# kije/HSLU_I.BA_RAYTRACING.F2501_raytracer

Hardware: AMD Instinct MI355X
Metric: Mray/s (primary+secondary, rays counted as the reference casts them), semesterbild@high_resolution (higher is better)
Workload: dtype f32; 1 GPU; semesterbild@high_resolution+anti_aliasing+soft_shadows (text.obj); width=1620, height=1350, rays_per_frame=34992000, rays_traced_per_frame=19683000, pixels_written=1768966, objects=14578, lights=50, parallelism=tiles48x48/1gpu, frames_in_flight=2, build_id=6bfb61b4c07ed2fe-p0s0w0o6, queue_bytes=0, scene_budget_bytes=2147483648, phases=0

## Files before the change

### hslu_i/ba_raytracing/f2501_raytracer_amd/csrc/rt_api.cpp

```cpp
#include <hip/hip_runtime.h>

#include <algorithm>
#include <chrono>
#include <cmath>
#include <cstdio>
#include <cstdlib>
#include <cstring>
#include <string>
#include <vector>

#include "rt_cell_prune.h"
#include "rt_host.h"

static void trace_point(hipStream_t stream, const char* what, uint32_t a = 0, uint32_t b = 0, uint32_t c = 0);
#define RC_TRY(expr) do { const int rc_ = (expr); if (rc_ != RT_OK) return rc_; } while (0)

extern "C" {

#ifndef RT_BUILD_ID
#define RT_BUILD_ID "unknown"
#endif
const char* rt_build_id(void) { return RT_BUILD_ID; }

int rt_selftest_exact_math(int device, const float* in, float* out_sqrt, float* out_rcp, uint32_t n) {
// ... 26 lines not shown
void rt_scene_destroy(rt_scene* s) {
  if (!s) return;
  (void)hipSetDevice(s->device);
  if (s->tables_ev) (void)hipEventDestroy(s->tables_ev);
  for (hipEvent_t e : s->frame_ev)
    if (e) (void)hipEventDestroy(e);
  for (auto& w : s->ws) {
    if (w.cnt_ev) (void)hipEventDestroy(w.cnt_ev);
    if (w.cnt_host) (void)hipHostFree(w.cnt_host);
    if (w.fork_ev) (void)hipEventDestroy(w.fork_ev);
    w.acc.release();
    for (auto& l : w.lane) {
      if (l.stream) (void)hipStreamSynchronize(l.stream), (void)hipStreamDestroy(l.stream);
      if (l.done_ev) (void)hipEventDestroy(l.done_ev);
      for (int k = 0; k < 2; k++) {
        if (l.shade_stream[k]) (void)hipStreamSynchronize(l.shade_stream[k]), (void)hipStreamDestroy(l.shade_stream[k]);
        if (l.shade_done[k]) (void)hipEventDestroy(l.shade_done[k]);
      }
      for (hipEvent_t e : l.level_ev) (void)hipEventDestroy(e);
      if (l.hit_ev) (void)hipEventDestroy(l.hit_ev);
      for (DevBuf* b : {&l.queues, &l.qcount, &l.trace_ws, &l.hard, &l.hitrec, &l.sets}) b->release();
    }
  }
  for (DevBuf* b : {&s->blob, &s->aa, &s->cloud, &s->counters, &s->suplist, &s->fb, &s->aux_rgb, &s->costmap, &s->aux_id, &s->aux_t, &s->flag_geo, &s->flags, &s->cell_lists, &s->progress_fb, &s->rays_argb})
    b->release();
  rt_scene_release_update(s);
  delete s;
}

static int upload(DevBuf& b, const void* src, size_t bytes) {
  int rc = b.ensure(bytes);
  if (rc != RT_OK) return rc;
  if (bytes) {
    hipError_t e = hipMemcpy(b.p, src, bytes, hipMemcpyHostToDevice);
    if (e != hipSuccess) return fail(RT_ERR_HIP, "hipMemcpy H2D failed: %s", hipGetErrorString(e));
  }
  return RT_OK;
}

int rt_scene_create(const rt_scene_desc* d, int device, rt_scene** out) {
  if (!d || !out) return fail(RT_ERR_INVALID_ARG, "null argument");
  *out = nullptr;
  int rc = rt_check_scene_desc(d);
  if (rc != RT_OK) return rc;
  if ((rc = rt_open_device(device)) != RT_OK) return rc;

  rt_scene* s = new rt_scene();
  s->device = device;
// ... 23 lines not shown
  s->n_tri_cells = pk.n_tri_cells;
  s->bytes_bvh = pk.bytes_bvh;
  s->max_leaf = pk.max_leaf;
  memcpy(s->aabb_lo, pk.aabb_lo, sizeof(s->aabb_lo));
  memcpy(s->aabb_hi, pk.aabb_hi, sizeof(s->aabb_hi));
  *out = s;
  return RT_OK;
}

int rt_scene_bvh_info(const rt_scene* s, rt_bvh_info* out) {
  if (!s || !out) return fail(RT_ERR_INVALID_ARG, "null argument");
  *out = s->info;
  return RT_OK;
}

int rt_scene_memory_info(const rt_scene* s, rt_scene_info* out) {
  if (!s || !out) return fail(RT_ERR_INVALID_ARG, "null argument");
  memset(out, 0, sizeof(*out));
  out->bytes_bvh = s->bytes_bvh;
  out->bytes_geometry = s->blob.cap > s->bytes_bvh ? s->blob.cap - s->bytes_bvh : 0;
  out->bytes_flags = s->flags.cap + s->flag_geo.cap;
  out->bytes_cell_lists = s->cell_lists.cap;
  out->bytes_tables = s->aa.cap + s->cloud.cap + s->counters.cap + s->suplist.cap + s->costmap.cap;
  for (const auto& w : s->ws) {
    out->bytes_workspace += w.bytes();
    for (const auto& l : w.lane) out->bytes_workspace += l.qcount.cap;
  }
  out->bytes_frames = s->fb.cap + s->aux_rgb.cap + s->aux_id.cap + s->aux_t.cap + s->progress_fb.cap + s->rays_argb.cap;
  out->bytes_total = out->bytes_geometry + out->bytes_bvh + out->bytes_flags + out->bytes_cell_lists + out->bytes_tables + out->bytes_workspace +
                     out->bytes_frames;
  out->budget_bytes = s->budget;
  out->n_receiver_cells = s->n_cells;
  out->cell_lists_built = s->cell_lists_built ? 1u : 0u;
  return RT_OK;
}

}

int rt_validate_params(const rt_params* p) {
  if (!p) return fail(RT_ERR_INVALID_ARG, "null params");
  if (p->abi_version != RT_ABI_VERSION)
    return fail(RT_ERR_INVALID_ARG, "rt_params.abi_version %u != %u", p->abi_version, RT_ABI_VERSION);
  if (p->width == 0 || p->height == 0) return fail(RT_ERR_INVALID_ARG, "empty frame");
  if ((uint64_t)p->width * p->height > 0x7FFFFFFFull) return fail(RT_ERR_INVALID_ARG, "frame too large");
  if (p->win_w && (p->win_x0 + (uint64_t)p->win_w > p->width || p->win_y0 + (uint64_t)p->win_h > p->height || !p->win_h))
    return fail(RT_ERR_INVALID_ARG, "window outside the frame");
// ... 90 lines not shown
  const size_t n = (size_t)p->n_cloud_sets * P->light_mult * 3;
  const bool new_table = s->cloud_host.size() != n || memcmp(s->cloud_host.data(), p->cloud_sets, n * 4) != 0;
  const bool new_scale = s->cloud_ball_f[0] != p->fw || s->cloud_ball_f[1] != p->fh || s->cloud_ball_f[2] != p->fd;
  if (new_table || new_scale) {
    RC_TRY(up.begin());
    RC_TRY(s->cloud.ensure(n / 3 * 16));
    if (new_table) s->cloud_host.assign(p->cloud_sets, p->cloud_sets + n);
    s->cloud_ball_f[0] = p->fw, s->cloud_ball_f[1] = p->fh, s->cloud_ball_f[2] = p->fd;
    rt_scale_cloud(s->cloud_host.data(), n, s->cloud_ball_f, &s->cloud_scaled, s->cloud_ball);
    HIP_TRY(hipMemcpyAsync(s->cloud.p, s->cloud_scaled.data(), n / 3 * 16, hipMemcpyHostToDevice, up.stream));
  }
  P->cloud_sets = (const float4*)s->cloud.p;
  memcpy(P->cloud_centre, s->cloud_ball, 12);
  P->cloud_delta = s->cloud_ball[3];
  rt_beam_constants(p->eps_distance, P);
  const uint32_t cap = p->tuning.shadow_candidate_cap;
  P->cand_cap = cap == RT_CAND_CAP_NONE ? 0u : (cap ? cap : 64u);
  return RT_OK;
}

static int prepare_receiver_flags(rt_scene* s, const rt_params* p, TableUpload& up, RtDevParams* P) {
  hipStream_t stream = up.stream;
  P->recv_flags = nullptr;
  if (p->tuning.no_receiver_flags || P->cand_cap == 0u) s->notes |= RT_NOTE_RECV_FLAGS_OFF_TUNING;
  if (!s->n_cells || !(P->cloud_delta > 0.0f)) s->notes |= RT_NOTE_RECV_FLAGS_OFF_SCENE;
  if (s->dev.n_lights > 8u) s->notes |= RT_NOTE_RECV_FLAGS_OFF_LIGHTS;
  if (p->traversal != RT_TRAVERSAL_BVH) s->notes |= RT_NOTE_RECV_FLAGS_OFF_TRAVERSAL;
  if (p->flags & RT_FLAG_BACKFACE_CULLING) s->notes |= RT_NOTE_RECV_FLAGS_OFF_CULLING;
  if (!p->tuning.no_receiver_flags && P->cand_cap != 0u && s->n_cells && s->dev.n_lights <= 8u && p->traversal == RT_TRAVERSAL_BVH &&
      !(p->flags & RT_FLAG_BACKFACE_CULLING) && P->cloud_delta > 0.0f) {
    const float key[8] = {P->beam_delta, p->eps_distance, P->cloud_centre[0], P->cloud_centre[1], P->cloud_centre[2], 1.f, 0.f, 0.f};
    if (memcmp(key, s->flags_key, sizeof(key)) != 0) {
      RC_TRY(up.begin());
      RtDevParams B = *P;
      B.flag_out = (uint16_t*)s->flags.p;
      B.flag_geo = (const float4*)s->flag_geo.p;
      B.n_cells = s->n_cells;
      B.n_tri_cells = s->n_tri_cells;
      s->cell_lists_built = false;
      B.cell_list_out = nullptr;
      const size_t list_bytes = (size_t)s->n_cells * s->dev.n_lights * 16u;
      size_t free_b = 0, total_b = 0;
      const size_t flag_bytes = s->flags.cap + s->flag_geo.cap;
      if (s->dev.n_slots <= 65533u && flag_bytes + list_bytes <= s->budget && hipMemGetInfo(&free_b, &total_b) == hipSuccess &&
          list_bytes <= (free_b + s->cell_lists.cap) / 4 && s->cell_lists.ensure(list_bytes + 64) == RT_OK) {
        HIP_TRY(hipMemsetAsync(s->cell_lists.p, 0xFF, list_bytes, stream));
        B.cell_list_out = (uint16_t*)s->cell_lists.p;
        s->cell_lists_built = true;
      }
      if (!s->cell_lists_built) s->cell_lists.release();
      hipError_t e = (hipError_t)rt_launch_flags(s->dev, B, stream);
      if (e != hipSuccess) return fail(RT_ERR_HIP, "rt_flags_kernel launch failed: %s", hipGetErrorString(e));
      trace_point(stream, "rt_flags_kernel: cells, lights, lists", s->n_cells, s->dev.n_lights, s->cell_lists_built ? 1u : 0u);
      static const char* const prune_env = getenv("RT_CELL_PRUNE");
      static const bool prune_off = prune_env && *prune_env == '0';
      if (s->cell_lists_built && !prune_off) {
        RtCellPruneArgs a{};
        a.flag_geo = (const float*)s->flag_geo.p;
        a.lists = (uint16_t*)s->cell_lists.p;
        a.flags = (uint16_t*)s->flags.p;
        a.n_cells = s->n_cells, a.n_tri_cells = s->n_tri_cells;
        memcpy(a.cloud_centre, P->cloud_centre, 12);
        a.beam_delta = P->beam_delta, a.beam_eps_o = P->beam_eps_o;
        a.mode = RT_PRUNE_FULL;
        e = (hipError_t)rt_launch_cell_prune(s->dev, a, stream);
        if (e != hipSuccess) return fail(RT_ERR_HIP, "rt_cell_prune_kernel launch failed: %s", hipGetErrorString(e));
        trace_point(stream, "rt_cell_prune_kernel: cells, lights", s->n_cells, s->dev.n_lights, 0u);
      }
      memcpy(s->flags_key, key, sizeof(key));
    }
    P->recv_flags = (const uint16_t*)s->flags.p;
    if (s->cell_lists_built && !p->tuning.no_cell_lists) P->cell_lists = (const uint4*)s->cell_lists.p;
  }
  if (!P->cell_lists) s->notes |= RT_NOTE_CELL_LISTS_OFF;
  return RT_OK;
}

static void copy_frame_shape(rt_scene* s, const rt_params* p, uint32_t* argb_dev, const rt_aux* aux_dev, RtDevParams* P) {
  P->max_depth_reflection = p->max_depth_reflection;
  P->max_depth_refraction = p->max_depth_refraction;
  s->sort_bits_wanted = p->tuning.sort_bits;
  s->lanes_wanted = p->tuning.sub_frames;
  s->phases_wanted = p->tuning.phases;
  s->levels_wanted = p->tuning.levels;
  if (p->win_w) {
    P->win_x0 = p->win_x0, P->win_y0 = p->win_y0, P->win_w = p->win_w, P->win_h = p->win_h;
  } else {
    P->win_x0 = P->win_y0 = 0;
    P->win_w = p->width;
    P->win_h = p->height;
// ... 782 lines not shown
```

### hslu_i/ba_raytracing/f2501_raytracer_amd/csrc/rt_cell_prune.h

```cpp
#pragma once

#include "rt_refit.h"

#define RT_PRUNE_LIST_SLOTS 8u
#define RT_PRUNE_LIST_END 0xFFFFu
#define RT_PRUNE_LIST_OVERFLOW 0xFFFEu
#define RT_PRUNE_G 8e-6f

#define RT_PRUNE_FAR 1u
#define RT_PRUNE_EUCLID 2u
#define RT_PRUNE_NO_RHO_WC 4u
#define RT_PRUNE_NO_RHO_FAR 8u
#define RT_PRUNE_FULL (RT_PRUNE_FAR | RT_PRUNE_EUCLID)

struct RtCellPruneArgs {
  const float* flag_geo;
  uint16_t* lists;
  uint16_t* flags;
  uint32_t n_cells, n_tri_cells;
  float cloud_centre[3];
  float beam_delta, beam_eps_o;
  uint32_t mode;
};

struct RtPruneBeam {
  float p[3], c[3], dseg[3];
  float rho, delta, lenp;
};

RT_HD static inline float rt_prune_dot(const float a[3], const float b[3]) {
  return rt_fadd(rt_fadd(rt_fmul(a[0], b[0]), rt_fmul(a[1], b[1])), rt_fmul(a[2], b[2]));
}
RT_HD static inline void rt_prune_cross(const float a[3], const float b[3], float out[3]) {
  out[0] = rt_fadd(rt_fmul(a[1], b[2]), -rt_fmul(a[2], b[1]));
  out[1] = rt_fadd(rt_fmul(a[2], b[0]), -rt_fmul(a[0], b[2]));
  out[2] = rt_fadd(rt_fmul(a[0], b[1]), -rt_fmul(a[1], b[0]));
}
RT_HD static inline void rt_prune_sub(const float a[3], const float b[3], float out[3]) {
  out[0] = rt_fadd(a[0], -b[0]), out[1] = rt_fadd(a[1], -b[1]), out[2] = rt_fadd(a[2], -b[2]);
}
RT_HD static inline float rt_prune_norm1(const float a[3]) { return rt_fadd(rt_fadd(fabsf(a[0]), fabsf(a[1])), fabsf(a[2])); }
RT_HD static inline float rt_prune_norm(const float a[3]) {
  const float q = rt_prune_dot(a, a);
  return q > 1e-30f ? rt_fmul(rt_fsqrt(q), 1.00001f) : rt_prune_norm1(a);
}
// ... 118 lines not shown
}

RT_HD static inline void rt_cell_prune_cell(const RtDevScene& sc, const char* base, const RtCellPruneArgs& a, uint32_t c, uint16_t* list, uint16_t* flag) {
  float pm[3], pt[8][3], extra;
  if (!rt_prune_cell_hull(sc, base, a, c, pm, pt, &extra)) return;
  float r = 0.0f, scale = rt_fadd(rt_prune_norm1(pm), extra);
  for (int k = 0; k < 8; k++) {
    float dk[3];
    rt_prune_sub(pt[k], pm, dk);
    r = fmaxf(r, rt_prune_norm(dk));
    scale = fmaxf(scale, rt_fadd(rt_prune_norm1(pt[k]), extra));
  }
  RtPruneBeam B;
  B.p[0] = pm[0], B.p[1] = pm[1], B.p[2] = pm[2];
  B.rho = rt_fadd(rt_fadd(rt_fmul(r, 1.0001f), rt_fmul(2e-6f, scale)), a.beam_eps_o);
  const float* lights = (const float*)(base + sc.off_lights);
  const float* isect = (const float*)(base + sc.off_tri_isect);
  uint32_t fl = *flag;
  bool fl_changed = false;
  for (uint32_t l = 0; l < sc.n_lights && l < 8u; l++) {
    uint16_t* w = list + (size_t)l * RT_PRUNE_LIST_SLOTS;
    uint16_t in[RT_PRUNE_LIST_SLOTS];
    memcpy(in, __builtin_assume_aligned(w, 16), 16);
    if (in[0] >= RT_PRUNE_LIST_OVERFLOW) continue;
    for (int x = 0; x < 3; x++) B.c[x] = rt_fadd(lights[8u * l + x], a.cloud_centre[x]);
    rt_prune_sub(B.c, B.p, B.dseg);
    B.delta = rt_fadd(a.beam_delta, rt_fmul(2e-6f, rt_fadd(scale, rt_prune_norm1(B.c))));
    B.lenp = rt_fadd(rt_fadd(rt_prune_norm(B.dseg), B.delta), B.rho);
    uint32_t n = 0, n_in = 0;
    uint16_t out[RT_PRUNE_LIST_SLOTS];
    for (uint32_t k = 0; k < RT_PRUNE_LIST_SLOTS; k++) {
      const uint32_t slot = in[k];
      if (slot >= RT_PRUNE_LIST_OVERFLOW) break;
      n_in++;
      if (slot < sc.n_slots && rt_prune_rule(B, isect + 12u * (size_t)slot, a.mode)) continue;
      out[n++] = (uint16_t)slot;
    }
    if (n == n_in) continue;
    for (uint32_t k = n; k < RT_PRUNE_LIST_SLOTS; k++) out[k] = (uint16_t)RT_PRUNE_LIST_END;
    memcpy(__builtin_assume_aligned(w, 16), out, 16);
    if (n == 0u) fl |= 1u << l, fl_changed = true;
  }
  if (fl_changed) *flag = (uint16_t)fl;
}

struct RtPackedScene;
void rt_cell_prune_packed(const RtPackedScene& pk, RtCellPruneArgs a);
int rt_launch_cell_prune(const RtDevScene& sc, const RtCellPruneArgs& a, void* stream);
```

### hslu_i/ba_raytracing/f2501_raytracer_amd/csrc/rt_host.h

```cpp
#pragma once

#include <hip/hip_runtime.h>

#include <string>
#include <vector>

#include "rt_ray_key.h"
#include "rt_scene_pack.h"

#define fail rt_fail

#define HIP_TRY(expr)                                                                          \
  do {                                                                                         \
    hipError_t e_ = (expr);                                                                    \
    if (e_ != hipSuccess)                                                                      \
      return fail(e_ == hipErrorOutOfMemory ? RT_ERR_OOM : RT_ERR_HIP, "%s failed: %s", #expr, \
                  hipGetErrorString(e_));                                                      \
  } while (0)

#define RT_SLOTS 4
#define RT_LANES 2
#define RT_MAX_DEPTH 64u

#define RT_CNT_OVERFLOW 0u
// ... 227 lines not shown
  uint32_t key_gen = 0;
  uint32_t sticky_notes = 0;
  bool stream_verified = false;
  uint32_t est[RT_LANES][RT_CNT_STRIDE] = {{0}};
  bool est_valid = false;
  uint32_t sort_bits_wanted = 0;
  uint32_t lanes_wanted = 0;
  uint32_t phases_wanted = 0;
  uint32_t levels_wanted = 0;
  uint32_t calm_frames = 1u << 30;
  uint32_t tables_version = 0;
  float aabb_lo[3] = {0.f, 0.f, 0.f}, aabb_hi[3] = {1.f, 1.f, 1.f};
  std::vector<float> aa_host, cloud_host, cloud_scaled;
  std::vector<uint32_t> aa_table;
  uint32_t aa_unique = 0;
  bool aa_dedup = true;
  hipEvent_t tables_ev = nullptr;
  hipStream_t tables_stream = nullptr, last_stream = nullptr;
  bool tables_pending = false, rendered = false;
  float cloud_ball[4] = {0.f, 0.f, 0.f, -1.f};
  DevBuf flag_geo, flags;
  DevBuf cell_lists;
  bool cell_lists_built = false;
  uint32_t n_cells = 0, n_tri_cells = 0;
  float flags_key[8] = {-1.f, 0.f, 0.f, 0.f, 0.f, 0.f, 0.f, 0.f};
  float cloud_ball_f[3] = {0.f, 0.f, 0.f};
  hipEvent_t frame_ev[RT_SLOTS] = {};
  bool frame_pending[RT_SLOTS] = {};
  uint32_t frame_seq[RT_SLOTS] = {};
  hipStream_t frame_stream[RT_SLOTS] = {};
  uint32_t frame_no = 0;
  int cur_block = 0, last_block = 0;
  int cur_ws = 0;
  int ws_last_block[RT_SLOTS] = {0, 1, 2, 3};
  uint32_t notes = 0;
  size_t queue_bytes = 0;
  RtRefitPlan plan;
  DevBuf plan_dev, upd_dev;
  size_t plan_off[5] = {0, 0, 0, 0, 0};
  void* upd_stage = nullptr;
  size_t upd_stage_cap = 0;
  float* upd_back = nullptr;
  uint64_t sah_created[2] = {0, 0};
  float sah_tri_cost = 2.0f;
  DevBuf sah_dev;
  uint32_t max_leaf = 4;
// ... 39 lines not shown
```

### hslu_i/ba_raytracing/f2501_raytracer_amd/csrc/rt_internal.h

```cpp
#pragma once

#include <stdint.h>

#include <vector>

#include "../../../../include/rt_hip.h"


struct RtNode {
  float lo0[3];
  uint32_t c0;
  float hi0[3];
  uint32_t n0;
  float lo1[3];
  uint32_t c1;
  float hi1[3];
  uint32_t n1;
};
static_assert(sizeof(RtNode) == 64, "node must be 64 bytes");

struct RtThrNode {
  float lo[3];
  uint32_t skip;
  float hi[3];
// ... 190 lines not shown
    case 10u: return lists ? RT_PRIMARY_SOFT10 : RT_PRIMARY_SOFT10_FLAGS;
    case 19u: return lists ? RT_PRIMARY_SOFT19 : RT_PRIMARY_SOFT19_FLAGS;
    case 28u: return lists ? RT_PRIMARY_SOFT28 : RT_PRIMARY_SOFT28_FLAGS;
    default: return RT_PRIMARY_GENERIC;
  }
}
static inline const char* rt_primary_variant_name(int v) {
  static const char* const names[RT_PRIMARY_VARIANTS] = {"rt_primary_kernel", "rt_primary_soft10_kernel", "rt_primary_soft19_kernel",
                                                         "rt_primary_soft28_kernel", "rt_primary_soft10_flags_kernel",
                                                         "rt_primary_soft19_flags_kernel", "rt_primary_soft28_flags_kernel"};
  return v >= 0 && v < RT_PRIMARY_VARIANTS ? names[v] : "";
}

uint32_t rt_primary_pixels_per_wg(const RtDevParams& p);
uint32_t rt_primary_total_wgs(const RtDevParams& p);
int rt_launch_primary(const RtDevScene& sc, const RtDevParams& p, uint32_t n_wgs, void* stream);
int rt_primary_variant_used(const RtDevScene& sc, const RtDevParams& p);
int rt_launch_trace(const RtDevScene& sc, const RtDevParams& p, uint32_t n_wgs, void* stream);
int rt_launch_sort(const RtDevParams& p, uint32_t n_wgs_place, void* stream);
int rt_launch_shade(const RtDevScene& sc, const RtDevParams& p, uint32_t n_wgs, void* stream);
int rt_launch_hard(const RtDevScene& sc, const RtDevParams& p, uint32_t n_wgs, void* stream);
int rt_launch_resolve(const RtDevParams& p, void* stream);
int rt_launch_flags(const RtDevScene& sc, const RtDevParams& p, void* stream);
int rt_launch_hit(const RtDevScene& sc, const RtDevParams& p, uint32_t n_wgs, void* stream);
int rt_launch_classify(const RtDevScene& sc, const RtDevParams& p, bool level0, uint32_t n_wgs, void* stream);
int rt_launch_compact(const RtDevParams& p, uint32_t n_wgs, void* stream);
int rt_launch_sets(const RtDevScene& sc, const RtDevParams& p, bool level0, int cls, uint32_t n_wgs, void* stream);
bool rt_has_cost_kernel();
bool rt_phases_arrive_inline();
int rt_launch_selftest_math(const float* in, float* out_sqrt, float* out_rcp, uint32_t n, void* stream);
int rt_launch_scatter(uint32_t* argb, const uint32_t* recv, const uint32_t* rank_off, const uint32_t* tile_slot, uint32_t width,
                      uint32_t height, uint32_t tile_size, uint32_t tiles_x, uint32_t n_ranks, void* stream);
```

### hslu_i/ba_raytracing/f2501_raytracer_amd/csrc/rt_kernels.hip

```cpp
#include <hip/hip_runtime.h>

#include <stdlib.h>

#include <type_traits>

#include "rt_internal.h"

#define RT_EPS 1.1920929e-7f

#define RT_OPAQUE(v) asm volatile("" : "+v"(v))
#define RT_OPAQUE_S(v) asm volatile("" : "+s"(v))
typedef const __attribute__((address_space(4))) char* rt_kernarg_ptr;
__device__ __forceinline__ rt_kernarg_ptr kernarg_fresh() {
  rt_kernarg_ptr p = (rt_kernarg_ptr)__builtin_amdgcn_kernarg_segment_ptr();
  asm volatile("" : "+s"(p));
  return p;
}
#define RT_KERNARG_OFF_P ((sizeof(RtDevScene) + alignof(RtDevParams) - 1) / alignof(RtDevParams) * alignof(RtDevParams))
static_assert(RT_KERNARG_OFF_P == 88, "RtDevParams follows RtDevScene at kernarg offset 88");
__device__ __forceinline__ const RtDevScene& kernarg_scene() { return *(const RtDevScene*)(const char*)kernarg_fresh(); }
__device__ __forceinline__ const RtDevParams& kernarg_params() {
  return *(const RtDevParams*)((const char*)kernarg_fresh() + RT_KERNARG_OFF_P);
}
#define wave_ballot(pred) __builtin_amdgcn_ballot_w64((bool)(pred))
// ... 668 lines not shown
    walk(std::true_type{});
  else
    walk(std::false_type{});
  return best;
}

#define RT_MAX_CANDIDATES 64u
#define RT_CAND_OVERFLOW 0xFFFFFFFFu

struct CandList {
  uint32_t reg;
  uint32_t count;
  uint32_t spheres;
  unsigned long long umbra;
#if RT_PROFILE == 5
  uint32_t own;
#endif
};

struct FatBeam {
  float r;
  V3 pt[8];
  uint16_t* list;
};
#define RT_CELL_LIST_SLOTS 8u
#define RT_CELL_LIST_END 0xFFFFu
#define RT_CELL_LIST_OVERFLOW 0xFFFEu
enum { COLLECT_OWN = 0, COLLECT_FLAGS = 1 };

template <bool CULL, int MODE = COLLECT_OWN, class C = CfgGeneric>
__device__ __forceinline__ CandList collect_light_candidates(const RtDevScene& sc, WaveCtx& W, bool alive, V3 p, V3 c,
                                                              const RtDevParams& P, V3 p_first, float p_spread, uint32_t cand_cap,
                                                              const FatBeam* fb = nullptr, bool walk_tris = true,
                                                              bool have_pre = false, uint32_t pre_reg = 0, uint32_t pre_count = 0) {
  RT_OPAQUE_S(cand_cap);
  const float delta = MODE == COLLECT_FLAGS ? P.beam_delta + fb->r : P.beam_delta;
  const float delta_e5 = MODE == COLLECT_FLAGS ? P.beam_delta_e5 + fb->r : P.beam_delta_e5;
  CandList L;
  L.reg = 0;
  L.count = 0;
  L.spheres = 0xFFFFFFFFu;
  L.umbra = 0ull;
#if RT_PROFILE == 5
  L.own = 0;
#endif
  const uint32_t lane_id = threadIdx.x & 63u;
  V3 dseg = c - p;
  float len = fmaxf(mag(dseg), 1e-20f);
  V3 inv = mk(clampf(__builtin_amdgcn_rcpf(dseg.x), -1e30f, 1e30f), clampf(__builtin_amdgcn_rcpf(dseg.y), -1e30f, 1e30f),
              clampf(__builtin_amdgcn_rcpf(dseg.z), -1e30f, 1e30f));
  V3 noi = mk(-(p.x * inv.x), -(p.y * inv.y), -(p.z * inv.z));
  V3 dl = mk(delta * fabsf(inv.x), delta * fabsf(inv.y), delta * fabsf(inv.z));
  float send = 1.0f + delta_e5 * __builtin_amdgcn_rcpf(len) + 1e-5f;
  float sbeg = -(delta_e5 * __builtin_amdgcn_rcpf(len) + 1e-5f);
  const V3 cn = noi - dl, cf = noi + dl;
  auto box = [&](const float* lo, const float* hi, float& smin) {
// ... 46 lines not shown
        rej &= wave_ballot(__builtin_fmaf(4e-6f, sk, __builtin_fmaf(X1, p_ulp, xk)) < rhs);
      }
    } else {
      rej = wave_ballot(__builtin_fmaf(4e-6f, st0, __builtin_fmaf(X1, p_ulp, xbs)) < t_push * (ad - dslack));
    }
    if (!(lanes & (open | ~rej))) return true;
    V3 y = mk((c2.y * dseg.z) + (-c2.z * dseg.y), (c2.z * dseg.x) + (-c2.x * dseg.z), (c2.x * dseg.y) + (-c2.y * dseg.x));
    float E2 = fabsf(c2.x) + fabsf(c2.y) + fabsf(c2.z);
    float ybs = __uint_as_float(__float_as_uint(dot(y, b)) ^ sgn);
    float su = E2 * geo;
    rej |= wave_ballot(ybs + su < 0.0f);
    if (!(lanes & (open | ~rej))) return true;
    V3 z = mk((dseg.y * c1.z) + (-dseg.z * c1.y), (dseg.z * c1.x) + (-dseg.x * c1.z), (dseg.x * c1.y) + (-dseg.y * c1.x));
    float E1 = fabsf(c1.x) + fabsf(c1.y) + fabsf(c1.z);
    float zbs = __uint_as_float(__float_as_uint(dot(z, b)) ^ sgn);
    float sv = E1 * geo;
    rej |= wave_ballot(zbs + sv < 0.0f) | wave_ballot((ybs + zbs) - ad - (su + sv) - dslack - 2e-6f * ad > 0.0f);
    if (!(lanes & (open | ~rej))) return true;
    if (MODE == COLLECT_FLAGS) {
      const lanemask surv = lanes & (open | ~rej);
      L.umbra |= surv;
      if (fb->list && lane_of(surv)) {
        if (L.reg < RT_CELL_LIST_SLOTS) fb->list[L.reg] = (uint16_t)slot;
        L.reg++;
      }
      return true;
    }
    if (!CULL && !(sload<uint32_t>(sc, sc.off_tri_id + slot * 4u) & RT_TRI_TRANSMISSIVE)) {
      const float dlo = ad - dslack;
      const float r_hi = lenp * __builtin_amdgcn_rcpf(dlo) * 1.00001f;
      const float r_lo = (len - delta) * __builtin_amdgcn_rcpf(ad + dslack) * 0.99999f;
      const float ex = __builtin_fmaf(4e-6f, st0, X1 * p_ulp);
      const float g_t = 2e-6f * (st0 + X1 * eps_o) * r_hi;
      const float t_lo = (xbs - ex) * r_lo - 1.001f * eps_o - g_t;
      const float t_hi = (xbs + ex) * r_hi + g_t;
      const lanemask inside = wave_ballot(ybs - su > 0.0f) & wave_ballot(zbs - sv > 0.0f) &
                              wave_ballot((ybs + zbs) + (su + sv) < dlo * 0.99999f) & wave_ballot(xbs > ex) & wave_ballot(t_lo > 2e-7f) &
                              wave_ballot(t_hi < (len - delta) - 1.01f * eps_o - 3e-7f * lenp) &
                              wave_ballot(dlo * rcp_lenp > __builtin_fmaf(2e-6f, X1, 2e-7f));
      L.umbra |= lanes & ~open & inside;
    }
#if RT_PROFILE == 5
    if (lane_of(lanes & (open | ~rej))) L.own++;
#endif
    return false;
  };
// ... 1283 lines not shown
    }
    if (any) {
      wrote = true;
      P1.argb[out_index(P1, pm2.gx, pm2.gy, pix)] = pack_argb(color);
      if (P1.aux_rgb) {
        P1.aux_rgb[3 * (size_t)pix + 0] = color.x;
        P1.aux_rgb[3 * (size_t)pix + 1] = color.y;
        P1.aux_rgb[3 * (size_t)pix + 2] = color.z;
      }
    }
  }
  if (COST && P1.cost_map && (threadIdx.x & 63u) == 0) {
    const unsigned long long dt = __builtin_readcyclecounter() - lds_cnt[16 + (threadIdx.x >> 6)];
    const uint32_t ppw = wave_local ? 4u * ppwave : 256u / n_thr;
    const uint32_t g = rt_batch_wg(P1, blockIdx.x) * ppw + (wave_local ? (threadIdx.x >> 6) * ppwave : threadIdx.x / n_thr), sup_slot = g >> 8;
    if (sup_slot < P1.n_sup) atomicAdd(&P1.cost_map[P1.sup_list ? P1.sup_list[sup_slot] : sup_slot], (uint32_t)(dt >> 6));
  }
  wave_flush(wv, P1, (uint32_t)__popcll(wave_ballot(wrote)), lds_cnt);
}

#ifndef RT_MIN_WAVES
#define RT_MIN_WAVES 6
#endif
__global__ __launch_bounds__(256, RT_MIN_WAVES) void rt_primary_kernel(RtDevScene sc, RtDevParams P) {
  __shared__ float4 lds_rgbh[256];
  __shared__ __attribute__((aligned(16))) float lds_stash[RT_STASH_FIX * 256];
  __shared__ unsigned long long lds_cnt[20];
  if (P.flags & RT_FLAG_BACKFACE_CULLING)
    primary_body<true, false>(sc, P, lds_rgbh, lds_stash, lds_cnt);
  else
    primary_body<false, false>(sc, P, lds_rgbh, lds_stash, lds_cnt);
}

#define RT_PRIMARY_SOFT_KERNEL(name, n, tables)                                                              \
  __global__ __launch_bounds__(256, RT_MIN_WAVES) void name(RtDevScene sc, RtDevParams P) {                  \
    __shared__ float4 lds_rgbh[256];                                                                         \
    __shared__ __attribute__((aligned(16))) float lds_stash[RT_STASH_FIX * 256];                             \
    __shared__ unsigned long long lds_cnt[20];                                                               \
    primary_body<false, false, false, false, CfgSoft<n, tables>>(sc, P, lds_rgbh, lds_stash, lds_cnt);       \
  }
RT_PRIMARY_SOFT_KERNEL(rt_primary_soft10_kernel, 10u, CFG_TABLES_LISTS)
RT_PRIMARY_SOFT_KERNEL(rt_primary_soft19_kernel, 19u, CFG_TABLES_LISTS)
RT_PRIMARY_SOFT_KERNEL(rt_primary_soft28_kernel, 28u, CFG_TABLES_LISTS)
RT_PRIMARY_SOFT_KERNEL(rt_primary_soft10_flags_kernel, 10u, CFG_TABLES_FLAGS)
RT_PRIMARY_SOFT_KERNEL(rt_primary_soft19_flags_kernel, 19u, CFG_TABLES_FLAGS)
RT_PRIMARY_SOFT_KERNEL(rt_primary_soft28_flags_kernel, 28u, CFG_TABLES_FLAGS)
// ... 407 lines not shown
  if (i >= P.win_w * P.win_h) return;
  const uint32_t gx = P.win_x0 + i % P.win_w, gy = P.win_y0 + i / P.win_w;
  const uint32_t pix = gy * P.width + gx;
  long long* a = P.acc + 4 * (size_t)pix;
  long long r = a[0], g = a[1], b = a[2], f = a[3];
  unsigned long long wrote = 0;
  if (f) {
    V3 c = mk((float)r * RT_ACC_INV_SCALE, (float)g * RT_ACC_INV_SCALE, (float)b * RT_ACC_INV_SCALE);
    P.argb[out_index(P, gx, gy, pix)] = pack_argb(c);
    if (P.aux_rgb) {
      P.aux_rgb[3 * (size_t)pix + 0] = c.x;
      P.aux_rgb[3 * (size_t)pix + 1] = c.y;
      P.aux_rgb[3 * (size_t)pix + 2] = c.z;
    }
    a[0] = a[1] = a[2] = a[3] = 0;
    wrote = 1;
  }
  if (P.resolve_counts_written && P.counters) {
    const uint32_t nw = (uint32_t)__popcll(wave_ballot(wrote != 0ull));
    if (nw && (threadIdx.x & 63u) == 0) atomicAdd(&P.counters[(size_t)(blockIdx.x % RT_COUNTER_REPLICAS) * 16u + 4u], (unsigned long long)nw);
  }
}

__global__ __launch_bounds__(256) void rt_flags_kernel(RtDevScene sc, RtDevParams P) {
  const uint32_t c = blockIdx.x * 256u + threadIdx.x;
  const bool have = c < P.n_cells;
  FatBeam fb;
  V3 pm = mk(0.0f, 0.0f, 0.0f);
  bool active = false;
  if (have && c < P.n_tri_cells) {
    uint32_t lo = 0u, hi = sc.n_triangles;
    while (hi - lo > 1u) {
      const uint32_t mid = (lo + hi) >> 1;
      if (__float_as_uint(P.flag_geo[3u * mid + 1u].w) <= c) lo = mid; else hi = mid;
    }
    const uint32_t t = lo;
    const float4 g0 = P.flag_geo[3u * t], g1 = P.flag_geo[3u * t + 1u], g2 = P.flag_geo[3u * t + 2u];
    const uint32_t R = __float_as_uint(g0.w), first = __float_as_uint(g1.w);
    const uint32_t local = c - first;
    const uint32_t j = R ? local / R : 0u, i = local - j * R;
    active = R != 0u && i + j < R;
    const V3 v1 = mk(g0.x, g0.y, g0.z), e1 = mk(g1.x, g1.y, g1.z), e2 = mk(g2.x, g2.y, g2.z);
    const float inv_r = R ? 1.0f / (float)R : 0.0f;
    const float u0 = ((float)i - 0.05f) * inv_r, u1 = ((float)i + 1.05f) * inv_r, w0 = ((float)j - 0.05f) * inv_r, w1 = ((float)j + 1.05f) * inv_r;
    fb.pt[0] = v1 + e1 * u0 + e2 * w0;
    fb.pt[1] = v1 + e1 * u1 + e2 * w0;
    fb.pt[2] = v1 + e1 * u0 + e2 * w1;
    fb.pt[3] = v1 + e1 * u1 + e2 * w1;
#pragma unroll
    for (int k = 0; k < 4; k++) fb.pt[4 + k] = fb.pt[k];
// ... 33 lines not shown
      }
      pm = ctr + uc * rad;
    }
  }
  if (!active) {
#pragma unroll
    for (int k = 0; k < 8; k++) fb.pt[k] = pm;
  }
  float r = 0.0f;
#pragma unroll
  for (int k = 0; k < 8; k++) {
    const V3 dk = fb.pt[k] - pm;
    r = fmaxf(r, fabsf(dk.x) + fabsf(dk.y) + fabsf(dk.z));
  }
  fb.r = __builtin_fmaf(r, 1.0001f, 4e-7f * (fabsf(pm.x) + fabsf(pm.y) + fabsf(pm.z)));
  WaveCtx W;
  W.n_nodes = W.n_tris = W.s_nodes = W.s_tris = W.s_passes = W.n_exact = W.s_exact = 0;
  W.o_exec = W.o_miss = 0;
  uint32_t flags = 0u;
  for (uint32_t l = 0; l < sc.n_lights && l < 8u; l++) {
    const float4 L0 = sload<float4>(sc, sc.off_lights + l * 32u);
    const V3 centre = mk(L0.x + P.cloud_centre[0], L0.y + P.cloud_centre[1], L0.z + P.cloud_centre[2]);
    fb.list = (P.cell_list_out && have) ? P.cell_list_out + ((size_t)c * sc.n_lights + l) * RT_CELL_LIST_SLOTS : nullptr;
    const CandList cl = collect_light_candidates<false, COLLECT_FLAGS>(sc, W, active, pm, centre, P, pm, 0.0f, RT_MAX_CANDIDATES, &fb,
                                                                          sc.n_triangles != 0u);
    if (fb.list && active && cl.reg > RT_CELL_LIST_SLOTS) fb.list[0] = (uint16_t)RT_CELL_LIST_OVERFLOW;
    const lanemask near_m = (lanemask)cl.count | ((lanemask)cl.spheres << 32);
    if (wave_ballot(active)) {
      flags |= lane_of(cl.umbra) ? 0u : (1u << l);
      flags |= lane_of(near_m) ? 0u : (1u << (8u + l));
    }
  }
  if (have) P.flag_out[c] = (uint16_t)(active ? flags : 0u);
}

__global__ __launch_bounds__(256) void rt_selftest_math_kernel(const float* in, float* out_sqrt, float* out_rcp, uint32_t n) {
  const uint32_t i = blockIdx.x * 256u + threadIdx.x;
  if (i >= n) return;
  out_sqrt[i] = exact_sqrt(in[i]);
  out_rcp[i] = exact_rcp(in[i]);
}

#include "rt_phases.h"
#include "rt_query.h"
#include "rt_rays.h"

}

bool rt_phases_arrive_inline() { return RT_ARRIVE_INLINE != 0; }
bool rt_has_cost_kernel() { return RT_COST_KERNEL != 0; }

int rt_launch_hit(const RtDevScene& sc, const RtDevParams& p, uint32_t n_wgs, void* stream) {
  if (n_wgs == 0) return 0;
  if (p.hit_spawns)
    hipLaunchKernelGGL(rt_hit_spawn_kernel, dim3(n_wgs), dim3(256), 0, (hipStream_t)stream, sc, p);
  else
    hipLaunchKernelGGL(rt_hit_kernel, dim3(n_wgs), dim3(256), 0, (hipStream_t)stream, sc, p);
  return (int)hipGetLastError();
}

int rt_launch_classify(const RtDevScene& sc, const RtDevParams& p, bool level0, uint32_t n_wgs, void* stream) {
  if (n_wgs == 0) {
    if (level0) return 0;
    n_wgs = 1;
  }
  if (level0)
    hipLaunchKernelGGL(rt_classify0_kernel, dim3(n_wgs), dim3(256), 0, (hipStream_t)stream, sc, p);
  else
    hipLaunchKernelGGL(rt_classify_kernel, dim3(n_wgs), dim3(256), 0, (hipStream_t)stream, sc, p);
  return (int)hipGetLastError();
}
// ... 112 lines not shown
  return (int)hipGetLastError();
}

int rt_launch_query_any(const RtDevScene& sc, const RtQueryArgs& q, void* stream) {
  if (q.n == 0) return 0;
  hipLaunchKernelGGL(rt_query_any_kernel, dim3(query_wgs(q.n)), dim3(256), 0, (hipStream_t)stream, sc, q);
  return (int)hipGetLastError();
}

int rt_launch_rays(const RtDevScene& sc, const RtDevParams& p, const RtRayArgs& r, uint32_t n_wgs, void* stream) {
  if (n_wgs == 0) return 0;
  if (p.acc)
    hipLaunchKernelGGL(rt_rays_stream_kernel, dim3(n_wgs), dim3(256), 0, (hipStream_t)stream, sc, p, r);
  else
    hipLaunchKernelGGL(rt_rays_kernel, dim3(n_wgs), dim3(256), 0, (hipStream_t)stream, sc, p, r);
  return (int)hipGetLastError();
}

int rt_launch_resolve(const RtDevParams& p, void* stream) {
  uint32_t n = p.win_w * p.win_h;
  hipLaunchKernelGGL(rt_resolve_kernel, dim3((n + 255u) / 256u), dim3(256), 0, (hipStream_t)stream, p);
  return (int)hipGetLastError();
}
```

Measured before the change: 8551 Mray/s.

## Spill overflowing shadow cell candidate lists into an extension pool for pruning

When a receiver cell's per-light candidate list overflows its 8 slots, the flags kernel now claims an entry in a device-side extension pool through an atomic counter and records up to 32 candidates there. The prune kernel reads these extended lists and, if the pruned set fits in 8 slots, writes it back as a compact list instead of leaving the cell marked overflow. The aim is to let more cells use precomputed short occluder lists in place of a full BVH shadow traversal. This costs extra one-time memory, atomics, and a separate kernel compilation unit, and the pool is freed once an event shows the prune has finished.

```diff
diff --git a/hslu_i/ba_raytracing/f2501_raytracer_amd/csrc/rt_api.cpp b/hslu_i/ba_raytracing/f2501_raytracer_amd/csrc/rt_api.cpp
--- a/hslu_i/ba_raytracing/f2501_raytracer_amd/csrc/rt_api.cpp
+++ b/hslu_i/ba_raytracing/f2501_raytracer_amd/csrc/rt_api.cpp
@@ -72,8 +72,9 @@
       for (DevBuf* b : {&l.queues, &l.qcount, &l.trace_ws, &l.hard, &l.hitrec, &l.sets}) b->release();
     }
   }
-  for (DevBuf* b : {&s->blob, &s->aa, &s->cloud, &s->counters, &s->suplist, &s->fb, &s->aux_rgb, &s->costmap, &s->aux_id, &s->aux_t, &s->flag_geo, &s->flags, &s->cell_lists, &s->progress_fb, &s->rays_argb})
+  for (DevBuf* b : {&s->blob, &s->aa, &s->cloud, &s->counters, &s->suplist, &s->fb, &s->aux_rgb, &s->costmap, &s->aux_id, &s->aux_t, &s->flag_geo, &s->flags, &s->cell_lists, &s->cell_ext, &s->progress_fb, &s->rays_argb})
     b->release();
+  if (s->cell_ext_ev) (void)hipEventDestroy(s->cell_ext_ev);
   rt_scene_release_update(s);
   delete s;
 }
@@ -143,6 +144,7 @@
   out->bytes_flags = s->flags.cap + s->flag_geo.cap;
   out->bytes_cell_lists = s->cell_lists.cap;
   out->bytes_tables = s->aa.cap + s->cloud.cap + s->counters.cap + s->suplist.cap + s->costmap.cap;
+  out->bytes_workspace += s->cell_ext.cap;
   for (const auto& w : s->ws) {
     out->bytes_workspace += w.bytes();
     for (const auto& l : w.lane) out->bytes_workspace += l.qcount.cap;
@@ -279,6 +281,7 @@
 static int prepare_receiver_flags(rt_scene* s, const rt_params* p, TableUpload& up, RtDevParams* P) {
   hipStream_t stream = up.stream;
   P->recv_flags = nullptr;
+  if (s->cell_ext.p && hipEventQuery(s->cell_ext_ev) == hipSuccess) s->cell_ext.release();
   if (p->tuning.no_receiver_flags || P->cand_cap == 0u) s->notes |= RT_NOTE_RECV_FLAGS_OFF_TUNING;
   if (!s->n_cells || !(P->cloud_delta > 0.0f)) s->notes |= RT_NOTE_RECV_FLAGS_OFF_SCENE;
   if (s->dev.n_lights > 8u) s->notes |= RT_NOTE_RECV_FLAGS_OFF_LIGHTS;
@@ -306,11 +309,31 @@
         s->cell_lists_built = true;
       }
       if (!s->cell_lists_built) s->cell_lists.release();
-      hipError_t e = (hipError_t)rt_launch_flags(s->dev, B, stream);
+      static const char* const prune_env = getenv("RT_CELL_PRUNE");
+      static const bool prune_off = prune_env && *prune_env == '0';
+      static const char* const ext_env = getenv("RT_CELL_EXT");
+      static const bool ext_off = ext_env && *ext_env == '0';
+      RtFlagsExt X{};
+      if (s->cell_lists_built && !prune_off && !ext_off) {
+        const size_t entry_bytes = RT_CELL_EXT_SLOTS * sizeof(uint16_t);
+        size_t room = s->budget - flag_bytes - list_bytes;
+        if (hipMemGetInfo(&free_b, &total_b) != hipSuccess) room = 0;
+        room = std::min(room, (free_b + s->cell_ext.cap) / 4);
+        const size_t entries = std::min({room / entry_bytes, (size_t)s->n_cells * s->dev.n_lights, (size_t)0xFFFFFFF0u});
+        if (entries && s->cell_ext.ensure(entries * entry_bytes + 256) == RT_OK) {
+          if (!s->cell_ext_ev) HIP_TRY(hipEventCreateWithFlags(&s->cell_ext_ev, hipEventDisableTiming));
+          HIP_TRY(hipMemsetAsync(s->cell_ext.p, 0xFF, entries * entry_bytes, stream));
+          X.pool = (uint16_t*)s->cell_ext.p;
+          X.counter = (uint32_t*)((char*)s->cell_ext.p + entries * entry_bytes);
+          X.entries = (uint32_t)entries, X.slots = RT_CELL_EXT_SLOTS;
+          HIP_TRY(hipMemsetAsync(X.counter, 0, sizeof(uint32_t), stream));
+        } else {
+          s->cell_ext.release();
+        }
+      }
+      hipError_t e = (hipError_t)rt_launch_flags_ext(s->dev, B, X, stream);
       if (e != hipSuccess) return fail(RT_ERR_HIP, "rt_flags_kernel launch failed: %s", hipGetErrorString(e));
       trace_point(stream, "rt_flags_kernel: cells, lights, lists", s->n_cells, s->dev.n_lights, s->cell_lists_built ? 1u : 0u);
-      static const char* const prune_env = getenv("RT_CELL_PRUNE");
-      static const bool prune_off = prune_env && *prune_env == '0';
       if (s->cell_lists_built && !prune_off) {
         RtCellPruneArgs a{};
         a.flag_geo = (const float*)s->flag_geo.p;
@@ -320,9 +343,11 @@
         memcpy(a.cloud_centre, P->cloud_centre, 12);
         a.beam_delta = P->beam_delta, a.beam_eps_o = P->beam_eps_o;
         a.mode = RT_PRUNE_FULL;
+        a.ext_pool = X.pool, a.ext_entries = X.entries, a.ext_slots = X.slots;
         e = (hipError_t)rt_launch_cell_prune(s->dev, a, stream);
         if (e != hipSuccess) return fail(RT_ERR_HIP, "rt_cell_prune_kernel launch failed: %s", hipGetErrorString(e));
-        trace_point(stream, "rt_cell_prune_kernel: cells, lights", s->n_cells, s->dev.n_lights, 0u);
+        trace_point(stream, "rt_cell_prune_kernel: cells, lights, pool entries", s->n_cells, s->dev.n_lights, X.entries);
+        if (X.pool) HIP_TRY(hipEventRecord(s->cell_ext_ev, stream));
       }
       memcpy(s->flags_key, key, sizeof(key));
     }
diff --git a/hslu_i/ba_raytracing/f2501_raytracer_amd/csrc/rt_cell_prune.h b/hslu_i/ba_raytracing/f2501_raytracer_amd/csrc/rt_cell_prune.h
--- a/hslu_i/ba_raytracing/f2501_raytracer_amd/csrc/rt_cell_prune.h
+++ b/hslu_i/ba_raytracing/f2501_raytracer_amd/csrc/rt_cell_prune.h
@@ -21,6 +21,8 @@
   float cloud_centre[3];
   float beam_delta, beam_eps_o;
   uint32_t mode;
+  const uint16_t* ext_pool;
+  uint32_t ext_entries, ext_slots;
 };
 
 struct RtPruneBeam {
@@ -185,21 +187,38 @@
     uint16_t* w = list + (size_t)l * RT_PRUNE_LIST_SLOTS;
     uint16_t in[RT_PRUNE_LIST_SLOTS];
     memcpy(in, __builtin_assume_aligned(w, 16), 16);
-    if (in[0] >= RT_PRUNE_LIST_OVERFLOW) continue;
+    if (in[0] == RT_PRUNE_LIST_END || (in[0] == RT_PRUNE_LIST_OVERFLOW && !a.ext_pool)) continue;
+    const uint16_t* ent = nullptr;
+    if (in[0] == RT_PRUNE_LIST_OVERFLOW) {
+      const uint32_t e = (uint32_t)in[2] | ((uint32_t)in[3] << 16);
+      if (e < a.ext_entries && a.ext_pool[(size_t)e * a.ext_slots] != RT_PRUNE_LIST_OVERFLOW) ent = a.ext_pool + (size_t)e * a.ext_slots;
+    }
+    const uint32_t n_cand = in[0] != RT_PRUNE_LIST_OVERFLOW ? RT_PRUNE_LIST_SLOTS : (ent ? a.ext_slots : 0u);
     for (int x = 0; x < 3; x++) B.c[x] = rt_fadd(lights[8u * l + x], a.cloud_centre[x]);
     rt_prune_sub(B.c, B.p, B.dseg);
     B.delta = rt_fadd(a.beam_delta, rt_fmul(2e-6f, rt_fadd(scale, rt_prune_norm1(B.c))));
     B.lenp = rt_fadd(rt_fadd(rt_prune_norm(B.dseg), B.delta), B.rho);
     uint32_t n = 0, n_in = 0;
     uint16_t out[RT_PRUNE_LIST_SLOTS];
-    for (uint32_t k = 0; k < RT_PRUNE_LIST_SLOTS; k++) {
-      const uint32_t slot = in[k];
+    bool fits = n_cand != 0u;
+    for (uint32_t k = 0; k < n_cand; k++) {
+      const uint32_t slot = ent ? ent[k] : in[k];
       if (slot >= RT_PRUNE_LIST_OVERFLOW) break;
       n_in++;
       if (slot < sc.n_slots && rt_prune_rule(B, isect + 12u * (size_t)slot, a.mode)) continue;
+      if (n == RT_PRUNE_LIST_SLOTS) {
+        fits = false;
+        break;
+      }
       out[n++] = (uint16_t)slot;
     }
-    if (n == n_in) continue;
+    if (in[0] == RT_PRUNE_LIST_OVERFLOW && !fits) {
+      out[0] = (uint16_t)RT_PRUNE_LIST_OVERFLOW;
+      for (uint32_t k = 1; k < RT_PRUNE_LIST_SLOTS; k++) out[k] = (uint16_t)RT_PRUNE_LIST_END;
+      memcpy(__builtin_assume_aligned(w, 16), out, 16);
+      continue;
+    }
+    if (n == n_in && !ent) continue;
     for (uint32_t k = n; k < RT_PRUNE_LIST_SLOTS; k++) out[k] = (uint16_t)RT_PRUNE_LIST_END;
     memcpy(__builtin_assume_aligned(w, 16), out, 16);
     if (n == 0u) fl |= 1u << l, fl_changed = true;
diff --git a/hslu_i/ba_raytracing/f2501_raytracer_amd/csrc/rt_flags_ext.hip b/hslu_i/ba_raytracing/f2501_raytracer_amd/csrc/rt_flags_ext.hip
--- /dev/null
+++ b/hslu_i/ba_raytracing/f2501_raytracer_amd/csrc/rt_flags_ext.hip
@@ -0,0 +1,2 @@
+#define RT_FLAGS_EXT_UNIT 1
+#include "rt_kernels.hip"
diff --git a/hslu_i/ba_raytracing/f2501_raytracer_amd/csrc/rt_host.h b/hslu_i/ba_raytracing/f2501_raytracer_amd/csrc/rt_host.h
--- a/hslu_i/ba_raytracing/f2501_raytracer_amd/csrc/rt_host.h
+++ b/hslu_i/ba_raytracing/f2501_raytracer_amd/csrc/rt_host.h
@@ -273,6 +273,8 @@
   DevBuf flag_geo, flags;
   DevBuf cell_lists;
   bool cell_lists_built = false;
+  DevBuf cell_ext;
+  hipEvent_t cell_ext_ev = nullptr;
   uint32_t n_cells = 0, n_tri_cells = 0;
   float flags_key[8] = {-1.f, 0.f, 0.f, 0.f, 0.f, 0.f, 0.f, 0.f};
   float cloud_ball_f[3] = {0.f, 0.f, 0.f};
diff --git a/hslu_i/ba_raytracing/f2501_raytracer_amd/csrc/rt_internal.h b/hslu_i/ba_raytracing/f2501_raytracer_amd/csrc/rt_internal.h
--- a/hslu_i/ba_raytracing/f2501_raytracer_amd/csrc/rt_internal.h
+++ b/hslu_i/ba_raytracing/f2501_raytracer_amd/csrc/rt_internal.h
@@ -236,6 +236,14 @@
 int rt_launch_hard(const RtDevScene& sc, const RtDevParams& p, uint32_t n_wgs, void* stream);
 int rt_launch_resolve(const RtDevParams& p, void* stream);
 int rt_launch_flags(const RtDevScene& sc, const RtDevParams& p, void* stream);
+#define RT_CELL_EXT_SLOTS 32u
+#define RT_CELL_EXT_NONE 0xFFFFFFFFu
+struct RtFlagsExt {
+  uint16_t* pool;
+  uint32_t* counter;
+  uint32_t entries, slots;
+};
+int rt_launch_flags_ext(const RtDevScene& sc, const RtDevParams& p, const RtFlagsExt& x, void* stream);
 int rt_launch_hit(const RtDevScene& sc, const RtDevParams& p, uint32_t n_wgs, void* stream);
 int rt_launch_classify(const RtDevScene& sc, const RtDevParams& p, bool level0, uint32_t n_wgs, void* stream);
 int rt_launch_compact(const RtDevParams& p, uint32_t n_wgs, void* stream);
diff --git a/hslu_i/ba_raytracing/f2501_raytracer_amd/csrc/rt_kernels.hip b/hslu_i/ba_raytracing/f2501_raytracer_amd/csrc/rt_kernels.hip
--- a/hslu_i/ba_raytracing/f2501_raytracer_amd/csrc/rt_kernels.hip
+++ b/hslu_i/ba_raytracing/f2501_raytracer_amd/csrc/rt_kernels.hip
@@ -714,16 +714,47 @@
   float r;
   V3 pt[8];
   uint16_t* list;
+  static constexpr bool EXT = false;
 };
+#ifdef RT_FLAGS_EXT_UNIT
+struct FatBeamExt : FatBeam {
+  RtFlagsExt ext;
+  static constexpr bool EXT = true;
+};
+#endif
 #define RT_CELL_LIST_SLOTS 8u
 #define RT_CELL_LIST_END 0xFFFFu
 #define RT_CELL_LIST_OVERFLOW 0xFFFEu
 enum { COLLECT_OWN = 0, COLLECT_FLAGS = 1 };
 
-template <bool CULL, int MODE = COLLECT_OWN, class C = CfgGeneric>
+#ifdef RT_FLAGS_EXT_UNIT
+__device__ __forceinline__ void flag_ext_put(const FatBeamExt& fb, uint32_t n, uint32_t slot) {
+  uint16_t* w = fb.list;
+  uint32_t e;
+  if (n == RT_CELL_LIST_SLOTS) {
+    e = atomicAdd(fb.ext.counter, 1u);
+    if (e >= fb.ext.entries) {
+      e = RT_CELL_EXT_NONE;
+    } else {
+      uint16_t* ent = fb.ext.pool + (size_t)e * fb.ext.slots;
+      for (uint32_t k = 0; k < RT_CELL_LIST_SLOTS; k++) ent[k] = w[k];
+    }
+    w[0] = (uint16_t)RT_CELL_LIST_OVERFLOW, w[2] = (uint16_t)(e & 0xFFFFu), w[3] = (uint16_t)(e >> 16);
+  } else {
+    e = (uint32_t)w[2] | ((uint32_t)w[3] << 16);
+  }
+  if (e >= fb.ext.entries) return;
+  uint16_t* ent = fb.ext.pool + (size_t)e * fb.ext.slots;
+  if (n < fb.ext.slots) ent[n] = (uint16_t)slot;
+  else ent[0] = (uint16_t)RT_CELL_LIST_OVERFLOW;
+}
+#endif
+
+template <bool CULL, int MODE = COLLECT_OWN, class C = CfgGeneric, class FB = FatBeam>
 __device__ __forceinline__ CandList collect_light_candidates(const RtDevScene& sc, WaveCtx& W, bool alive, V3 p, V3 c,
                                                               const RtDevParams& P, V3 p_first, float p_spread, uint32_t cand_cap,
-                                                              const FatBeam* fb = nullptr, bool walk_tris = true,
+                                                              const typename std::enable_if<true, FB>::type* fb = nullptr,
+                                                              bool walk_tris = true,
                                                               bool have_pre = false, uint32_t pre_reg = 0, uint32_t pre_count = 0) {
   RT_OPAQUE_S(cand_cap);
   const float delta = MODE == COLLECT_FLAGS ? P.beam_delta + fb->r : P.beam_delta;
@@ -816,6 +847,9 @@
       L.umbra |= surv;
       if (fb->list && lane_of(surv)) {
         if (L.reg < RT_CELL_LIST_SLOTS) fb->list[L.reg] = (uint16_t)slot;
+        if constexpr (FB::EXT) {
+          if (L.reg >= RT_CELL_LIST_SLOTS) flag_ext_put(*fb, L.reg, slot);
+        }
         L.reg++;
       }
       return true;
@@ -2145,6 +2179,7 @@
 #ifndef RT_MIN_WAVES
 #define RT_MIN_WAVES 6
 #endif
+#ifndef RT_FLAGS_EXT_UNIT
 __global__ __launch_bounds__(256, RT_MIN_WAVES) void rt_primary_kernel(RtDevScene sc, RtDevParams P) {
   __shared__ float4 lds_rgbh[256];
   __shared__ __attribute__((aligned(16))) float lds_stash[RT_STASH_FIX * 256];
@@ -2598,10 +2633,12 @@
   }
 }
 
-__global__ __launch_bounds__(256) void rt_flags_kernel(RtDevScene sc, RtDevParams P) {
+#endif
+
+template <class FB>
+__device__ __forceinline__ void flags_cell(const RtDevScene& sc, const RtDevParams& P, FB& fb) {
   const uint32_t c = blockIdx.x * 256u + threadIdx.x;
   const bool have = c < P.n_cells;
-  FatBeam fb;
   V3 pm = mk(0.0f, 0.0f, 0.0f);
   bool active = false;
   if (have && c < P.n_tri_cells) {
@@ -2681,7 +2718,7 @@
     const float4 L0 = sload<float4>(sc, sc.off_lights + l * 32u);
     const V3 centre = mk(L0.x + P.cloud_centre[0], L0.y + P.cloud_centre[1], L0.z + P.cloud_centre[2]);
     fb.list = (P.cell_list_out && have) ? P.cell_list_out + ((size_t)c * sc.n_lights + l) * RT_CELL_LIST_SLOTS : nullptr;
-    const CandList cl = collect_light_candidates<false, COLLECT_FLAGS>(sc, W, active, pm, centre, P, pm, 0.0f, RT_MAX_CANDIDATES, &fb,
+    const CandList cl = collect_light_candidates<false, COLLECT_FLAGS, CfgGeneric, FB>(sc, W, active, pm, centre, P, pm, 0.0f, RT_MAX_CANDIDATES, &fb,
                                                                           sc.n_triangles != 0u);
     if (fb.list && active && cl.reg > RT_CELL_LIST_SLOTS) fb.list[0] = (uint16_t)RT_CELL_LIST_OVERFLOW;
     const lanemask near_m = (lanemask)cl.count | ((lanemask)cl.spheres << 32);
@@ -2693,6 +2730,12 @@
   if (have) P.flag_out[c] = (uint16_t)(active ? flags : 0u);
 }
 
+#ifndef RT_FLAGS_EXT_UNIT
+__global__ __launch_bounds__(256) void rt_flags_kernel(RtDevScene sc, RtDevParams P) {
+  FatBeam fb;
+  flags_cell(sc, P, fb);
+}
+
 __global__ __launch_bounds__(256) void rt_selftest_math_kernel(const float* in, float* out_sqrt, float* out_rcp, uint32_t n) {
   const uint32_t i = blockIdx.x * 256u + threadIdx.x;
   if (i >= n) return;
@@ -2704,8 +2747,17 @@
 #include "rt_query.h"
 #include "rt_rays.h"
 
-}
-
+#else
+__global__ __launch_bounds__(256) void rt_flags_ext_kernel(RtDevScene sc, RtDevParams P, RtFlagsExt X) {
+  FatBeamExt fb;
+  fb.ext = X;
+  flags_cell(sc, P, fb);
+}
+#endif
+
+}
+
+#ifndef RT_FLAGS_EXT_UNIT
 bool rt_phases_arrive_inline() { return RT_ARRIVE_INLINE != 0; }
 bool rt_has_cost_kernel() { return RT_COST_KERNEL != 0; }
 
@@ -2864,3 +2916,13 @@
   hipLaunchKernelGGL(rt_resolve_kernel, dim3((n + 255u) / 256u), dim3(256), 0, (hipStream_t)stream, p);
   return (int)hipGetLastError();
 }
+
+#else
+int rt_launch_flags_ext(const RtDevScene& sc, const RtDevParams& p, const RtFlagsExt& x, void* stream) {
+  if (!x.pool) return rt_launch_flags(sc, p, stream);
+  if (p.n_cells == 0) return 0;
+  if (!x.counter || !p.cell_list_out || x.slots < 16u || x.slots > 64u || (x.slots & 7u)) return (int)hipErrorInvalidValue;
+  hipLaunchKernelGGL(rt_flags_ext_kernel, dim3((p.n_cells + 255u) / 256u), dim3(256), 0, (hipStream_t)stream, sc, p, x);
+  return (int)hipGetLastError();
+}
+#endif
```

Measured after the change: 8623 Mray/s (median of 6 runs). Within noise of the previous version (+0.8%).
